# magneano/shyft

Measured on NVIDIA B200. Metric: cell-timesteps/sec (pt_gs_k run_cells), higher is better.
Workload: dtype f64

## Files before the change

### shyft_b200/csrc/sb2_capi.cu

```cuda
#include <cuda_runtime.h>

#include <cstdio>
#include <cstdlib>
#include <cstring>
#include <map>
#include <mutex>
#include <memory>
#include <string>
#include <type_traits>
#include <vector>

#include "../../include/shyft_b200.h"
#include "sb2_host.hpp"
#include "sb2_interp.cuh"
#include "sb2_ptgsk.cuh"
#include "sb2_hbv.cuh"
#include "sb2_ptssk.cuh"
#include "sb2_pthpsk.cuh"
#include "sb2_routing.cuh"
#include <nvtx3/nvToolsExt.h>
#include "sb2_unit.cuh"
#include "sb2_goal.cuh"
#include "sb2_stats.cuh"

// ... 532 lines not shown
        nvtxRangePop();
        m->launches += 3;
    } else {
        const dim3 grid((unsigned)(groups * n_slices), ne);
        zero_tickets();
        if (m->stack == SB2_PT_SS_K) {
            SskRunArgs a{};
            common(a);
            a.params = m->d_ssk_params.p;
            a.inv_dt_hours = make_inv_divisor(a.dt_hours);
            a.step_in_days = a.dt_seconds / 86400.0;
            a.collect = collect & 15;
            ptssk_run_kernel<<<grid, SB2_BLOCK, SB2_MTAB_BYTES, m->stream>>>(a);
        } else if (m->stack == SB2_PT_HPS_K) {
            HpsRunArgs a{};
            common(a);
            a.params = m->d_hps_params.p;
            a.bb0 = 0.98 * 5.670373e-8 * sb_pow4(273.15);
            a.inv_dt_seconds = make_inv_divisor(a.dt_seconds);
            a.ens_params = t.hps_members; a.ens_state_stride = t.state_stride; a.ens_partial_stride = t.partial_stride; a.ens_resp_stride = t.resp_stride;
            a.collect = collect & 15;
            if (t.hps_members) pthpsk_run_kernel<true><<<grid, SB2_BLOCK, SB2_MTAB_BYTES, m->stream>>>(a);
            else pthpsk_run_kernel<false><<<grid, SB2_BLOCK, SB2_MTAB_BYTES, m->stream>>>(a);
        } else {
            HbvRunArgs a{};
            common(a);
            a.params = m->d_hbv_params.p;
            a.inv_dt_hours = make_inv_divisor(a.dt_hours);
            a.step_in_days = a.dt_seconds / 86400.0;
            a.par0 = make_hbv_param(m->stack == SB2_HBV_STACK, m->region_param.data());
            a.ens_params = t.hbv_members; a.ens_state_stride = t.state_stride; a.ens_partial_stride = t.partial_stride; a.ens_resp_stride = t.resp_stride;
            a.collect = collect & 15;
            if (m->stack == SB2_PT_HS_K) {
                if (upar) hbv_run_kernel<false, true><<<grid, SB2_BLOCK, SB2_MTAB_BYTES, m->stream>>>(a);
                else hbv_run_kernel<false, false><<<grid, SB2_BLOCK, SB2_MTAB_BYTES, m->stream>>>(a);
            } else {
                if (upar) hbv_run_kernel<true, true><<<grid, SB2_BLOCK, SB2_MTAB_BYTES, m->stream>>>(a);
                else hbv_run_kernel<true, false><<<grid, SB2_BLOCK, SB2_MTAB_BYTES, m->stream>>>(a);
            }
        }
        ++m->launches;
    }
    CUDA_OK(cudaGetLastError());
    NvtxRange nv_reduce("catchment_reduce");
    const int64_t total = int64_t(chunk) * m->n_catch();
    catchment_reduce_kernel<<<dim3((unsigned)grid_for(total, 256), ne), 256, 0, m->stream>>>(
        t.partial, m->n_slots, m->d_cat_ptr.p, m->d_cat_slots.p, int(m->n_catch()), chunk, t.cq, t.cc, s0, t.partial_stride, t.catch_stride);
    CUDA_OK(cudaGetLastError());
    ++m->launches;
}

void launch_step_range(sb2_model* m, int64_t first, int64_t n_steps, bool collect_end_state) {
    sync_parameters(m);
    sync_filter(m);
    const int64_t n = m->n;
    if (m->partial_steps == 0) {
        constexpr int64_t cap = 4096, scratch_gb = 16;
        int64_t ps = std::max<int64_t>(1, std::min<int64_t>(cap, (int64_t(cap / 4) << 20) / std::max<int64_t>(1, m->n_slots * 16)));
        if (m->stack == SB2_PT_GS_K) ps = std::max<int64_t>(16, std::min<int64_t>(ps, (scratch_gb << 30) / (40 * std::max<int64_t>(1, n))));
        m->partial_steps = int(ps);
        m->d_partial.resize(size_t(ps) * m->n_slots * 2);
    }
    if (m->stack == SB2_PT_GS_K)
        for (auto& b : m->d_scr) b.ensure(size_t(std::min<int64_t>(m->partial_steps, n_steps)) * n);
    m->d_tickets.ensure(size_t(1 + step_groups(m)));
    StepTarget t;
    t.state = m->d_state.p; t.partial = m->d_partial.p; t.cq = m->d_cq.p; t.cc = m->d_cc.p; t.scr = m->d_scr;
    t.tickets = m->d_tickets.p;
    t.series = true;
    const int64_t n_chunks = std::max<int64_t>(1, (n_steps + m->partial_steps - 1) / m->partial_steps);
    int64_t even = (n_steps + n_chunks - 1) / n_chunks;
    even = std::min<int64_t>(m->partial_steps, (even + 127) / 128 * 128);
    for (int64_t done = 0; done < n_steps; done += even) {
        const int chunk = int(std::min<int64_t>(even, n_steps - done));
        launch_step_chunk(m, t, first + done, chunk, collect_end_state && done + chunk >= n_steps);
    }
}

void check_device_errors(sb2_model* m) {
    int flag = 0;
    CUDA_OK(cudaMemcpyAsync(&flag, m->d_error_flag.p, sizeof(int), cudaMemcpyDeviceToHost, m->stream));
    CUDA_OK(cudaStreamSynchronize(m->stream));
    if (flag) {
        CUDA_OK(cudaMemsetAsync(m->d_error_flag.p, 0, sizeof(int), m->stream));
        if (flag & ERR_KIRCHNER_STEP) throw Error("Max number of iterations exceeded (500). A new step size was not found.");
        if (flag & ERR_HBV_NEGATIVE_OUTFLOW) throw Error("hbv_snow: Negative outflow");
        if (flag & ERR_SKAUGEN_SEARCH) throw Error("skaugen: sca_rel_red found no root (boost::math::tools::bisect: no change of sign) or the gamma density overflowed");
        throw Error("device error flag " + std::to_string(flag));
    }
}

void validate_run_args(const sb2_model* m, int start_step, int n_steps) {
    if (!(m->T > 0)) throw Error("region_model::run with invalid time_axis invoked");
    if (start_step < 0 || int64_t(start_step) + 1 > m->T) throw Error("region_model::run start_step must in range[0..n_steps-1>");
    if (n_steps < 0) throw Error("region_model::run n_steps must be range[0..time-axis-steps]");
    if (int64_t(start_step) + n_steps > m->T) throw Error("region_model::run start_step+n_steps must be within time-axis range");
}
void snapshot_initial_state_if_unset(sb2_model* m) {
    if (m->has_initial) return;
    m->d_initial_state.resize(m->d_state.n);
    CUDA_OK(cudaMemcpyAsync(m->d_initial_state.p, m->d_state.p, m->d_state.n * sizeof(double), cudaMemcpyDeviceToDevice, m->stream));
    m->has_initial = true;
}

IdwParam to_idw(const sb2_idw_parameter& q) {
    IdwParam p{};
    p.max_members = int(q.max_members);
    p.max_distance = q.max_distance;
    p.distance_measure_factor = q.distance_measure_factor;
    p.zscale = q.zscale;
    p.default_temp_gradient = q.default_temp_gradient;
    p.scale_factor = q.scale_factor;
    p.gradient_by_equation = q.gradient_by_equation;
    return p;
}
const sb2_idw_parameter& idw_parameter_of(const sb2_interpolation_parameter& ip, int var) {
    switch (var) {
        case SB2_TEMPERATURE: return ip.temperature_idw;
        case SB2_PRECIPITATION: return ip.precipitation;
        case SB2_RADIATION: return ip.radiation;
        case SB2_WIND_SPEED: return ip.wind_speed;
        default: return ip.rel_hum;
    }
}
int idw_kind_of(int var) {
    switch (var) {
        case SB2_TEMPERATURE: return IDW_TEMPERATURE;
        case SB2_PRECIPITATION: return IDW_PRECIPITATION;
        case SB2_RADIATION: return IDW_RADIATION;
        case SB2_WIND_SPEED: return IDW_WIND_SPEED;
        default: return IDW_REL_HUM;
    }
}

void build_idw_plan(sb2_model* m, int var) {
    IdwPlan& pl = m->idw[var];
    const Source& s = m->src[var];
    pl.p = to_idw(idw_parameter_of(m->ip, var));
    if (pl.p.max_members < 1) throw Error("inverse_distance: max_members must be >= 1");
    pl.n_src = s.n_src;
    const size_t k = size_t(std::min<int64_t>(pl.p.max_members, s.n_src));
    pl.idx.resize(k * m->n); pl.w.resize(k * m->n); pl.f.resize(k * m->n); pl.cnt.resize(m->n);
    const double d2 = pl.p.max_distance * pl.p.max_distance;
    const double min_weight = 1.0 / sb_pow(d2, pl.p.distance_measure_factor / 2.0);
    idw_build_neighbours_kernel<<<grid_for(m->n, 128), 128, 0, m->stream>>>(idw_kind_of(var), m->n, m->d_x.p, m->d_y.p, m->d_z.p, m->d_slope.p,
                                                                           int(s.n_src), s.d_xyz.p, pl.p, min_weight, pl.idx.p, pl.w.p, pl.f.p,
                                                                           pl.cnt.p);
    CUDA_OK(cudaGetLastError());
    ++m->launches;
    pl.valid = true;
    pl.dense_valid = false;
}

int idw_tile_steps(int64_t n_src) {
    const int64_t budget = 32 * 1024 / 8;
    return int(std::max<int64_t>(1, std::min<int64_t>(64, budget / std::max<int64_t>(1, n_src))));
}

void run_idw(sb2_model* m, int var, int64_t first, int64_t n_steps, double* out) {
    IdwPlan& pl = m->idw[var];
    if (!pl.valid) build_idw_plan(m, var);
    const Source& s = m->src[var];
    if (!s.has_nonfinite && !(var == SB2_TEMPERATURE && pl.p.gradient_by_equation) && s.n_src <= 96 && !m->force_sparse_idw) {
        if (!pl.dense_valid) {
            pl.dense.resize(size_t(s.n_src) * m->n);
            pl.addc.resize(size_t(m->n));
            idw_build_dense_kernel<<<grid_for(m->n, 128), 128, 0, m->stream>>>(idw_kind_of(var), m->n, int(s.n_src), m->d_z.p, pl.p.default_temp_gradient,
                                                                              pl.idx.p, pl.w.p, pl.f.p, pl.cnt.p, pl.dense.p, pl.addc.p);
            CUDA_OK(cudaGetLastError());
            ++m->launches;
            const int nvp = int(s.n_src);
            const int ks = nvp <= 16 ? 4 : (nvp <= 32 ? 8 : (nvp <= 64 ? 16 : 24)), ntile = nvp <= 32 ? 4 : (nvp <= 64 ? 2 : 1);
            const int64_t n_tiles = grid_for(m->n, 32 * ntile) * 4;
            pl.ulist.resize(size_t(n_tiles) * ks * 4);
            pl.ukc.resize(size_t(n_tiles));
            CUDA_OK(cudaMemsetAsync(pl.ukc.p, 0, size_t(n_tiles), m->stream));
            idw_union_plan_kernel<<<grid_for(n_tiles * 32, 128), 128, 0, m->stream>>>(m->n, nvp, pl.dense.p, 8 * ntile, ks * 4, pl.ulist.p, pl.ukc.p);
            CUDA_OK(cudaGetLastError());
            ++m->launches;
            std::vector<uint8_t> h_kc(size_t(n_tiles), 0);
            CUDA_OK(cudaMemcpyAsync(h_kc.data(), pl.ukc.p, h_kc.size(), cudaMemcpyDeviceToHost, m->stream));
            CUDA_OK(cudaStreamSynchronize(m->stream));
            pl.kc_max = 0;
            for (uint8_t k : h_kc) pl.kc_max = std::max(pl.kc_max, int(k));
            pl.dense_valid = true;
        }
        const int nv = int(s.n_src);
        const double* v = s.d_values.p + first * s.n_src;
        const int use_tma = (nv % 2 == 0 && (reinterpret_cast<uintptr_t>(v) & 15) == 0) ? 1 : 0;
#define SB2_DENSE(KS, NT, KROW, TS)                                                                                                       \
    do {                                                                                                                                  \
        const int smem = dense_smem_bytes(KROW, TS);                                                                                      \
        auto kern = dense_apply_dmma_kernel<KS, NT, 0, true, KROW, TS>;                                                                   \
        CUDA_OK(cudaFuncSetAttribute(kern, cudaFuncAttributeMaxDynamicSharedMemorySize, smem));                                           \
        kern<<<grid_for(m->n, 32 * NT), 128, smem, m->stream>>>(m->n, nullptr, nv, pl.dense.p, pl.addc.p, nullptr, v, s.n_src, nullptr,   \
                                                                int(n_steps), m->d_active.p, out, pl.ulist.p, pl.ukc.p, use_tma,          \
                                                                4 * (nv <= 16 ? 4 : (nv <= 32 ? 8 : (nv <= 64 ? 16 : 24))));              \
    } while (0)
        if (nv <= 16) SB2_DENSE(4, 4, 4, 0);
        else if (nv <= 32) SB2_DENSE(8, 4, 8, 0);
        else if (nv <= 64) {
            if (pl.kc_max <= 4) SB2_DENSE(4, 2, 16, SB2_DENSE_TILE_COMPACT);
            else if (pl.kc_max <= 6) SB2_DENSE(6, 2, 16, SB2_DENSE_TILE_COMPACT);
            else if (pl.kc_max <= 8) SB2_DENSE(8, 2, 16, SB2_DENSE_TILE_COMPACT);
            else if (pl.kc_max <= 10) SB2_DENSE(10, 2, 16, SB2_DENSE_TILE_COMPACT);
            else if (pl.kc_max <= 12) SB2_DENSE(12, 2, 16, SB2_DENSE_TILE_COMPACT);
            else SB2_DENSE(16, 2, 16, 0);
        } else SB2_DENSE(24, 1, 24, 0);
#undef SB2_DENSE
        CUDA_OK(cudaGetLastError());
        ++m->launches;
        return;
    }
    const int tile = idw_tile_steps(s.n_src);
    const int max_k = int(std::max<int64_t>(1, std::min<int64_t>(pl.p.max_members, s.n_src)));
    const size_t smem = size_t(tile) * s.n_src * sizeof(double) + size_t(max_k) * IDW_BLOCK * (2 * sizeof(double) + sizeof(int));
    if (smem > 200 * 1024) throw Error("inverse_distance: too many sources / members for the shared-memory tiles");
    const int g = grid_for(m->n, IDW_BLOCK);
#define SB2_IDW(K)                                                                                                                   \
    {                                                                                                                                \
        if (smem > 48 * 1024) CUDA_OK(cudaFuncSetAttribute(idw_apply_kernel<K>, cudaFuncAttributeMaxDynamicSharedMemorySize, int(smem))); \
        idw_apply_kernel<K><<<g, IDW_BLOCK, smem, m->stream>>>(m->n, m->d_z.p, int(s.n_src), s.d_xyz.p, s.d_values.p, first, int(n_steps),  \
                                                               pl.p, pl.idx.p, pl.w.p, pl.f.p, pl.cnt.p, m->d_active.p, out, tile, max_k);     \
    }
    switch (idw_kind_of(var)) {
        case IDW_TEMPERATURE: SB2_IDW(IDW_TEMPERATURE) break;
        case IDW_PRECIPITATION: SB2_IDW(IDW_PRECIPITATION) break;
        case IDW_RADIATION: SB2_IDW(IDW_RADIATION) break;
        case IDW_WIND_SPEED: SB2_IDW(IDW_WIND_SPEED) break;
        default: SB2_IDW(IDW_REL_HUM) break;
    }
#undef SB2_IDW
    CUDA_OK(cudaGetLastError());
    ++m->launches;
}

BtkOps* btk_ops_for(sb2_model* m, const std::vector<int>& valid, bool check_rank) {
    for (auto& o : m->btk_cache)
        if (o->valid == valid) return o.get();
    if (m->btk_cache.size() >= 8) m->btk_cache.erase(m->btk_cache.begin() + 1);
    const Source& s = m->src[SB2_TEMPERATURE];
    const sb2_btk_parameter& bp = m->ip.temperature;
    host::BtkStationOps h = host::btk_station_ops(s.xyz, valid, bp.sill, bp.nug, bp.range, bp.zscale, bp.gradient_sd, check_rank);
    auto o = std::make_unique<BtkOps>();
    o->valid = valid;
    const int nv = int(valid.size());
    std::vector<double> sub_xyz(size_t(nv) * 3);
    for (int i = 0; i < nv; ++i)
        for (int c = 0; c < 3; ++c) sub_xyz[3 * i + c] = s.xyz[3 * valid[i] + c];
    DevArray<double> d_sub_xyz, d_Kinv, d_FtKinv, d_M22;
    d_sub_xyz.upload(sub_xyz, m->stream);
    d_Kinv.upload(h.K_inv.a, m->stream);
    d_FtKinv.upload(h.FtKinv.a, m->stream);
    d_M22.upload(h.M22.a, m->stream);
    o->E_beta_w.upload(h.E_beta_w.a, m->stream);
    o->sz.upload(h.z, m->stream);
    std::vector<int32_t> vi(valid.begin(), valid.end());
    o->valid_idx.upload(vi, m->stream);
    o->omega.resize(size_t(nv) * m->n);
    o->bm.resize(size_t(2) * m->n);
    m->d_btk_kbuf.ensure(size_t(nv) * m->n);
    btk_build_operators_kernel<<<grid_for(m->n, 128), 128, 0, m->stream>>>(m->n, m->d_x.p, m->d_y.p, m->d_z.p, nv, d_sub_xyz.p, d_Kinv.p,
                                                                          d_FtKinv.p, d_M22.p, bp.sill - bp.nug, bp.range, bp.zscale,
                                                                          o->omega.p, o->bm.p, m->d_btk_kbuf.p);
    CUDA_OK(cudaGetLastError());
    ++m->launches;
    CUDA_OK(cudaStreamSynchronize(m->stream));
    m->btk_cache.push_back(std::move(o));
    return m->btk_cache.back().get();
}

void run_btk(sb2_model* m, int64_t first, int64_t n_steps, double* out) {
    const Source& s = m->src[SB2_TEMPERATURE];
    const int S = int(s.n_src);
    std::vector<int> all(S);
    for (int i = 0; i < S; ++i) all[i] = i;
    BtkOps* full = btk_ops_for(m, all, true);
    int64_t i = 0;
    while (i < n_steps) {
        std::vector<int> valid;
        if (!s.has_nonfinite) valid = all;
        else {
            const double* v = &s.h_values[size_t(first + i) * S];
            for (int k = 0; k < S; ++k) if (std::isfinite(v[k])) valid.push_back(k);
        }
        if (valid.empty()) throw Error("bayesian kriging temperature: No valid sources for time period, giving up.");
        int64_t j = i + 1;
        if (!s.has_nonfinite) j = n_steps;
        else
            for (; j < n_steps; ++j) {
                const double* v = &s.h_values[size_t(first + j) * S];
                bool same = true;
                size_t q = 0;
                for (int k = 0; k < S && same; ++k) {
                    const bool fin = std::isfinite(v[k]);
                    const bool was = q < valid.size() && valid[q] == k;
                    if (fin != was) same = false;
                    if (was) ++q;
                }
                if (!same) break;
            }
        BtkOps* op = int(valid.size()) == S ? full : btk_ops_for(m, valid, false);
        const int nv = int(valid.size());
        const int64_t seg = j - i;
        m->d_btk_beta.ensure(size_t(seg) * 2);
        m->d_btk_resid.ensure(size_t(seg) * nv);
        btk_step_prepare_kernel<<<grid_for(seg, 128), 128, 0, m->stream>>>(int(seg), first + i, S, s.d_values.p, op->valid_idx.p, nv,
                                                                          op->E_beta_w.p, op->sz.p, m->d_btk_beta.p, m->d_btk_resid.p);
        CUDA_OK(cudaGetLastError());
        double* o = out + i * m->n;
        const double* pri = m->d_prior_gradient.p + first + i;
        const int use_tma = (nv % 2 == 0 && (reinterpret_cast<uintptr_t>(m->d_btk_resid.p) & 15) == 0) ? 1 : 0;
#define SB2_BTK(KS, NT, TS)                                                                                                               \
    do {                                                                                                                                  \
        const int smem = dense_smem_bytes(KS, TS);                                                                                        \
        auto kern = dense_apply_dmma_kernel<KS, NT, 1, false, KS, TS>;                                                                    \
        CUDA_OK(cudaFuncSetAttribute(kern, cudaFuncAttributeMaxDynamicSharedMemorySize, smem));                                           \
        kern<<<grid_for(m->n, 32 * NT), 128, smem, m->stream>>>(m->n, m->d_z.p, nv, op->omega.p, op->bm.p, m->d_btk_beta.p,               \
                                                                m->d_btk_resid.p, nv, pri, int(seg), m->d_active.p, o, nullptr, nullptr,  \
                                                                use_tma, 0);                                                              \
    } while (0)
        if (nv <= 16) SB2_BTK(4, 4, 0);
        else if (nv <= 32) SB2_BTK(8, 4, 0);
        else if (nv <= 64) SB2_BTK(16, 2, 0);
        else if (nv <= 96) SB2_BTK(24, 1, 0);
        else {
            const int tile = idw_tile_steps(nv);
            const size_t smem = size_t(tile) * nv * sizeof(double);
            btk_apply_kernel<<<grid_for(m->n, 128), 128, smem, m->stream>>>(m->n, m->d_z.p, nv, op->omega.p, op->bm.p, m->d_btk_beta.p,
                                                                           m->d_btk_resid.p, pri, int(seg), m->d_active.p, o, tile);
        }
#undef SB2_BTK
        CUDA_OK(cudaGetLastError());
        m->launches += 2;
        i = j;
    }
}

void interpolate_variable(sb2_model* m, int var, int64_t first, int64_t n_steps, double* out) {
    const Source& s = m->src[var];
    if (s.n_src == 0) return;
    if (var == SB2_TEMPERATURE) {
        if (s.n_src > 1) {
            if (m->ip.use_idw_for_temperature) run_idw(m, var, first, n_steps, out);
            else run_btk(m, first, n_steps, out);
        } else {
            broadcast_source_kernel<<<grid_for(m->n, 128), 128, 0, m->stream>>>(m->n, s.d_values.p + first, int(n_steps), m->d_active.p, out);
            CUDA_OK(cudaGetLastError());
            ++m->launches;
        }
    } else run_idw(m, var, first, n_steps, out);
}

bool interpolate_range(sb2_model* m, int64_t first, int64_t n_steps, int best_effort) {
    NvtxRange nv("interpolate");
    sync_filter(m);
    bool all_ok = true;
    for (int var = 0; var < SB2_N_FORCING; ++var) {
        try {
            interpolate_variable(m, var, first, n_steps, m->d_forcing[var].p + (first - m->forcing_first) * m->n);
        } catch (const std::exception&) {
            if (!best_effort) throw;
            all_ok = false;
        }
    }
    return all_ok;
}

void set_interpolation_parameter(sb2_model* m, const sb2_interpolation_parameter* ip) {
    if (!ip) throw Error("null interpolation parameter");
    if (m->ip_valid && std::memcmp(&m->ip, ip, sizeof(*ip)) == 0) return;
    m->ip = *ip;
    m->ip_valid = true;
    for (auto& pl : m->idw) pl.valid = false;
    m->btk_cache.clear();
}

void ensure_forcing(sb2_model* m, int64_t first, int64_t rows, bool nan_fill) {
    if (m->forcing_first == first && m->forcing_rows == rows && m->d_forcing[0].p) return;
    for (auto& f : m->d_forcing) f.resize(size_t(rows) * m->n);
    m->forcing_first = first;
    m->forcing_rows = rows;
    if (nan_fill)
        for (auto& f : m->d_forcing) fill_nan(m, f.p, rows * m->n);
}

void copy_out_2d(sb2_model* m, const double* d_src , int64_t rows, double* out, int layout) {
    if (layout == SB2_TIME_MAJOR) {
        CUDA_OK(cudaMemcpyAsync(out, d_src, size_t(rows) * m->n * sizeof(double), cudaMemcpyDeviceToHost, m->stream));
    } else {
        DevArray<double> tmp;
        tmp.resize(size_t(rows) * m->n);
        dim3 b(32, 8), g((unsigned)((m->n + 31) / 32), (unsigned)((rows + 31) / 32));
        transpose_kernel<<<g, b, 0, m->stream>>>(d_src, tmp.p, rows, m->n);
        CUDA_OK(cudaGetLastError());
        ++m->launches;
        CUDA_OK(cudaMemcpyAsync(out, tmp.p, size_t(rows) * m->n * sizeof(double), cudaMemcpyDeviceToHost, m->stream));
        CUDA_OK(cudaStreamSynchronize(m->stream));
        return;
    }
    CUDA_OK(cudaStreamSynchronize(m->stream));
}

void time_begin(sb2_model* m, int which) { CUDA_OK(cudaEventRecord(m->ev[which], m->stream)); }
float time_end(sb2_model* m, int a, int b) {
    CUDA_OK(cudaEventRecord(m->ev[b], m->stream));
    CUDA_OK(cudaEventSynchronize(m->ev[b]));
    float ms = 0.f;
    CUDA_OK(cudaEventElapsedTime(&ms, m->ev[a], m->ev[b]));
    return ms;
}
void ensure_routing_plan(sb2_model* m) {
    if (m->route) return;
    if (m->rivers.empty()) throw Error("routing: the river network is empty");
    const int off = kStacks[m->stack].routing_velocity;
    std::vector<double> cell_routing(size_t(m->n) * 5);
    for (int64_t i = 0; i < m->n; ++i) {
        auto f = m->catch_param.find(m->geo[i].catchment_id);
        const std::vector<double>& p = f != m->catch_param.end() ? f->second : m->region_param;
        double* cr = &cell_routing[5 * i];
        cr[0] = double(m->geo[i].routing_id); cr[1] = m->geo[i].routing_distance;
        cr[2] = p[off]; cr[3] = p[off + 1]; cr[4] = p[off + 2];
    }
    m->route = build_routing_plan(m->rivers, cell_routing, m->n, m->dt, m->stream);
}


void build_goal_targets(sb2_model* m, std::vector<GoalTarget>& gt, const double* cq, const double* cc, int64_t ens_stride) {
    gt.clear();
    int first_kind = -1;
    for (auto& tp : m->targets)
        if (first_kind < 0 && (tp->property == SB2_TARGET_DISCHARGE || tp->property == SB2_TARGET_CELL_CHARGE)) first_kind = tp->property;
    for (auto& tp : m->targets) {
        sb2_model::Target& t = *tp;
        GoalTarget g{};
        g.obs = t.d_obs.p;
        g.first_step = (t.t0 - m->t0) / m->dt;
        g.steps_per_period = int32_t(t.dt / m->dt);
        g.n = int32_t(t.obs.size());
        g.calc_mode = (t.calc_mode == SB2_GOAL_ABS_DIFF && t.property == SB2_TARGET_CELL_CHARGE) ? GOAL_ABS_DIFF_SCALED : t.calc_mode;
        g.s_r = t.s_r; g.s_a = t.s_a; g.s_b = t.s_b;
        g.dt_seconds = double(m->dt) / 1e6;
        g.rows = m->T;
        g.scale = nullptr;
        if (t.property == SB2_TARGET_DISCHARGE || t.property == SB2_TARGET_CELL_CHARGE) {
            g.series = first_kind == SB2_TARGET_DISCHARGE ? cq : cc;
            g.ens_stride = ens_stride;
            g.n_col = int32_t(m->n_catch());
            g.cix = t.d_cix.p;
            g.n_cix = int32_t(t.cids.size());
        } else {
            g.series = t.d_series.p;
            g.ens_stride = 0;
            g.n_col = 1;
            g.cix = t.d_cix.p;
            g.n_cix = 1;
        }
        if (!t.aligned) {
            if (ens_stride != 0) throw Error("target_specification: batched evaluation needs target axes aligned with the model axis");
            const int64_t T = m->T, n = int64_t(t.obs.size());
            if (!m->d_axis_t.p || int64_t(m->d_axis_t.n) != T) {
                std::vector<int64_t> tt(static_cast<size_t>(T), 0);
                for (int64_t i = 0; i < T; ++i) tt[size_t(i)] = m->t0 + i * m->dt;
                m->d_axis_t.upload(tt, m->stream);
            }
            DevArray<double> d_prop, d_a, d_b;
            d_prop.resize(size_t(T));
            t.d_projected.resize(size_t(n));
            auto project = [&](int mode, double* out) {
                goal_property_kernel<<<grid_for(T, 256), 256, 0, m->stream>>>(g.series, T, g.n_col, g.cix, g.n_cix, mode, d_prop.p);
                if (t.points.empty())
                    average_accessor_kernel<<<grid_for(n, 256), 256, 0, m->stream>>>(m->d_axis_t.p, d_prop.p, T, 1, m->t0 + T * m->dt, 0, t.t0, t.dt, n, out);
                else
// ... 1400 lines not shown
```

### shyft_b200/csrc/sb2_interp.cuh

```cuda
#pragma once
#include <stdint.h>

#include "sb2_math.cuh"

namespace sb2 {

enum { IDW_TEMPERATURE = 0, IDW_PRECIPITATION = 1, IDW_RADIATION = 2, IDW_WIND_SPEED = 3, IDW_REL_HUM = 4 };

struct IdwParam {
    int max_members;
    double max_distance, distance_measure_factor, zscale, default_temp_gradient, scale_factor;
    int gradient_by_equation;
};

__device__ __forceinline__ double distance_measure(double ax, double ay, double az, double bx, double by, double bz, double p, double zscale) {
    const double dx = __dsub_rn(ax, bx), dy = __dsub_rn(ay, by), dz = __dsub_rn(az, bz);
    const double d2 = __dadd_rn(__dadd_rn(__dmul_rn(dx, dx), __dmul_rn(dy, dy)), __dmul_rn(__dmul_rn(__dmul_rn(dz, dz), zscale), zscale));
    const double e = p / 2.0;
    return sb_pow(d2, e);
}

__global__ void idw_build_neighbours_kernel(int kind, int64_t n_cells, const double* __restrict__ cx, const double* __restrict__ cy,
                                            const double* __restrict__ cz, const double* __restrict__ cslope, int n_src,
                                            const double* __restrict__ sxyz, IdwParam p, double min_weight, int32_t* __restrict__ nb_idx,
// ... 82 lines not shown
    double* sf = sw + (size_t)max_k * IDW_BLOCK;
    int* sk = (int*)(sf + (size_t)max_k * IDW_BLOCK);
    const int tid = threadIdx.x;
    const int64_t c = (int64_t)blockIdx.x * blockDim.x + tid;
    const bool ok = c < n_cells && (active == nullptr || active[c] != 0);
    const int cnt = ok ? nb_n[c] : 0;
    const double z = ok ? cz[c] : 0.0;
    for (int j = 0; j < cnt; ++j) {
        sk[j * IDW_BLOCK + tid] = nb_idx[(int64_t)j * n_cells + c];
        sw[j * IDW_BLOCK + tid] = nb_w[(int64_t)j * n_cells + c];
        sf[j * IDW_BLOCK + tid] = nb_f[(int64_t)j * n_cells + c];
    }
    for (int t0 = 0; t0 < n_steps; t0 += tile_steps) {
        const int nt = min(tile_steps, n_steps - t0);
        __syncthreads();
        for (int e = tid; e < nt * n_src; e += blockDim.x) sv[e] = src[(first_step + t0) * n_src + e];
        __syncthreads();
        if (!ok) continue;
        for (int i = 0; i < nt; ++i) {
            const double* v = sv + i * n_src;
            double scale = 1.0;
            if (KIND == IDW_TEMPERATURE) {
                scale = p.default_temp_gradient;
                int nv = 0, mn = -1, mx = -1, first[4] = {-1, -1, -1, -1};
                double zmn = 0, zmx = 0;
                for (int j = 0; j < cnt; ++j) {
                    const int k = sk[j * IDW_BLOCK + tid];
                    if (!isfinite(v[k])) continue;
                    const double h = sf[j * IDW_BLOCK + tid];
                    if (nv < 4) first[nv] = k;
                    if (nv == 0) { mn = mx = k; zmn = zmx = h; }
                    else if (h < zmn) { mn = k; zmn = h; }
                    else if (h > zmx) { mx = k; zmx = h; }
                    ++nv;
                }
                bool solved = false;
                if (p.gradient_by_equation && nv > 3) {
                    double A[3][3], b[3], x[3];
                    for (int r = 0; r < 3; ++r) {
                        A[r][0] = sxyz[3 * first[r + 1]] - sxyz[3 * first[0]];
                        A[r][1] = sxyz[3 * first[r + 1] + 1] - sxyz[3 * first[0] + 1];
                        A[r][2] = sxyz[3 * first[r + 1] + 2] - sxyz[3 * first[0] + 2];
                        b[r] = v[first[r + 1]] - v[first[0]];
                    }
                    if (solve3(A, b, x)) { scale = x[2]; solved = true; }
                }
                if (!solved && nv > 1) {
                    const double dz = zmx - zmn;
                    scale = dz > 50.0 ? (v[mx] - v[mn]) / dz : p.default_temp_gradient;
                }
            }
            double sum_w = 0, sum_wv = 0;
            for (int j = 0; j < cnt; ++j) {
                const double s = v[sk[j * IDW_BLOCK + tid]];
                if (isfinite(s)) {
                    const double w = sw[j * IDW_BLOCK + tid];
                    double tv;
                    if (KIND == IDW_TEMPERATURE) tv = s + scale * (z - sf[j * IDW_BLOCK + tid]);
                    else if (KIND == IDW_PRECIPITATION || KIND == IDW_RADIATION) tv = s * sf[j * IDW_BLOCK + tid];
                    else tv = s;
                    sum_wv += w * tv;
                    sum_w += w;
                }
            }
            out[(int64_t)(t0 + i) * n_cells + c] = sum_wv / sum_w;
        }
    }
}

__global__ void btk_build_operators_kernel(int64_t n_cells, const double* __restrict__ cx, const double* __restrict__ cy,
                                           const double* __restrict__ cz, int n_src, const double* __restrict__ sxyz,
                                           const double* __restrict__ K_inv, const double* __restrict__ FtKinv,
                                           const double* __restrict__ M22, double sill_m_nug, double range, double zscale,
                                           double* __restrict__ omega , double* __restrict__ bm ,
                                           double* __restrict__ kbuf ) {
    const int64_t c = (int64_t)blockIdx.x * blockDim.x + threadIdx.x;
    if (c >= n_cells) return;
    const double x = cx[c], y = cy[c], z = cz[c];
    for (int s = 0; s < n_src; ++s) {
        const double dx = sxyz[3 * s] - x, dy = sxyz[3 * s + 1] - y, dz = sxyz[3 * s + 2] - z;
        const double d = sqrt(dx * dx + dy * dy + dz * dz * zscale * zscale);
        kbuf[(int64_t)s * n_cells + c] = sill_m_nug * sb_exp(-d / range);
    }
    double g0 = 0.0, g1 = 0.0;
    for (int j = 0; j < n_src; ++j) {
        const double kj = kbuf[(int64_t)j * n_cells + c];
        g0 += FtKinv[j] * kj;
        g1 += FtKinv[n_src + j] * kj;
    }
    const double d0 = 1.0 - g0, d1 = z - g1;
    bm[c] = d0 * M22[0] + d1 * M22[2];
    bm[n_cells + c] = d0 * M22[1] + d1 * M22[3];
    for (int s = 0; s < n_src; ++s) {
        double acc = 0.0;
        for (int j = 0; j < n_src; ++j) acc += kbuf[(int64_t)j * n_cells + c] * K_inv[j * n_src + s];
        omega[(int64_t)s * n_cells + c] = acc;
    }
}

__global__ void btk_step_prepare_kernel(int n_steps, int64_t first_step, int n_src, const double* __restrict__ src,
                                        const int32_t* __restrict__ valid_idx, int n_valid, const double* __restrict__ E_beta_w ,
                                        const double* __restrict__ sz_valid, double* __restrict__ beta ,
                                        double* __restrict__ resid ) {
    const int i = blockIdx.x * blockDim.x + threadIdx.x;
    if (i >= n_steps) return;
    const double* v = src + (first_step + i) * n_src;
    double b0 = 0.0, b1 = 0.0;
    for (int s = 0; s < n_valid; ++s) {
        const double t = v[valid_idx[s]];
        b0 += E_beta_w[s] * t;
        b1 += E_beta_w[n_valid + s] * t;
    }
    beta[2 * i] = b0;
    beta[2 * i + 1] = b1;
    for (int s = 0; s < n_valid; ++s) resid[(int64_t)i * n_valid + s] = v[valid_idx[s]] - (1.0 * b0 + sz_valid[s] * b1);
}

__global__ void __launch_bounds__(128) btk_apply_kernel(int64_t n_cells, const double* __restrict__ cz, int n_valid,
                                                        const double* __restrict__ omega , const double* __restrict__ bm,
                                                        const double* __restrict__ beta, const double* __restrict__ resid,
                                                        const double* __restrict__ prior_gradient , int n_steps,
                                                        const uint8_t* __restrict__ active, double* __restrict__ out ,
                                                        int tile_steps) {
    extern __shared__ double sr[];
    const int64_t c = (int64_t)blockIdx.x * blockDim.x + threadIdx.x;
    const bool ok = c < n_cells && (active == nullptr || active[c] != 0);
    const double z = ok ? cz[c] : 0.0, bm0 = ok ? bm[c] : 0.0, bm1 = ok ? bm[n_cells + c] : 0.0;
    for (int t0 = 0; t0 < n_steps; t0 += tile_steps) {
        const int nt = min(tile_steps, n_steps - t0);
        __syncthreads();
        for (int e = threadIdx.x; e < nt * n_valid; e += blockDim.x) sr[e] = resid[(int64_t)t0 * n_valid + e];
        __syncthreads();
        if (!ok) continue;
        for (int i = 0; i < nt; ++i) {
            const double b0 = beta[2 * (t0 + i)], b1 = beta[2 * (t0 + i) + 1];
            double acc = 0.0;
            for (int s = 0; s < n_valid; ++s) acc += omega[(int64_t)s * n_cells + c] * sr[i * n_valid + s];
            const double t_hat = (1.0 * b0 + z * b1) + acc;
            out[(int64_t)(t0 + i) * n_cells + c] = t_hat - (bm0 * (b0 - 0.0) + bm1 * (b1 - prior_gradient[t0 + i]));
        }
    }
}

__device__ __forceinline__ void dmma_m8n8k4(double& d0, double& d1, double a, double b) {
    asm volatile("mma.sync.aligned.m8n8k4.row.col.f64.f64.f64.f64 {%0,%1}, {%2}, {%3}, {%0,%1};" : "+d"(d0), "+d"(d1) : "d"(a), "d"(b));
}
__device__ __forceinline__ uint32_t smem_u32(const void* p) { return (uint32_t)__cvta_generic_to_shared(p); }
__device__ __forceinline__ void mbar_init(unsigned long long* bar, int count) {
    asm volatile("mbarrier.init.shared::cta.b64 [%0], %1;" ::"r"(smem_u32(bar)), "r"(count));
}
__device__ __forceinline__ void mbar_arrive_expect_tx(unsigned long long* bar, uint32_t bytes) {
    asm volatile("mbarrier.arrive.expect_tx.shared::cta.b64 _, [%0], %1;" ::"r"(smem_u32(bar)), "r"(bytes) : "memory");
}
__device__ __forceinline__ void bulk_copy_g2s(void* dst, const void* src, uint32_t bytes, unsigned long long* bar) {
    asm volatile("cp.async.bulk.shared::cluster.global.mbarrier::complete_tx::bytes [%0], [%1], %2, [%3];" ::"r"(smem_u32(dst)), "l"(src), "r"(bytes),
                 "r"(smem_u32(bar))
                 : "memory");
}
__device__ __forceinline__ void mbar_wait(unsigned long long* bar, uint32_t parity) {
    uint32_t done = 0;
    for (int spins = 0; !done; ++spins) {
        asm volatile("{\n.reg .pred p;\nmbarrier.try_wait.parity.shared::cta.b64 p, [%1], %2;\nselp.u32 %0, 1, 0, p;\n}" : "=r"(done) : "r"(smem_u32(bar)), "r"(parity) : "memory");
        if (spins > (1 << 24)) __trap();
    }
}

__host__ __device__ constexpr int dense_tile_steps(int krow, int tile_steps) { return tile_steps > 0 ? tile_steps : (krow > 16 ? 32 : 64); }
__host__ __device__ constexpr int dense_smem_bytes(int krow, int tile_steps) { return 2 * dense_tile_steps(krow, tile_steps) * (krow * 4 + 4) * 8; }
template <int KSTEPS, int NT, int MODE, bool COMPACT, int KROW = KSTEPS, int TILE_STEPS = 0>
__global__ void __launch_bounds__(128) dense_apply_dmma_kernel(int64_t n_cells, const double* __restrict__ cz, int n_valid,
                                                               const double* __restrict__ omega , const double* __restrict__ bm,
                                                               const double* __restrict__ beta ,
                                                               const double* __restrict__ resid , int64_t row_stride,
                                                               const double* __restrict__ prior_gradient , int n_steps,
                                                               const uint8_t* __restrict__ active, double* __restrict__ out ,
                                                               const int32_t* __restrict__ ulist, const uint8_t* __restrict__ ukc, int use_tma,
                                                               int ul_stride ) {
    constexpr int KP = KROW * 4 + 4;
    constexpr int TILE = dense_tile_steps(KROW, TILE_STEPS);
    extern __shared__ __align__(16) double sr_dyn[];
    __shared__ double sbeta[2][TILE * 2];
    __shared__ double spri[2][TILE];
    __shared__ __align__(8) unsigned long long bar[2];
    const int lane = threadIdx.x & 31, warp = threadIdx.x >> 5;
    const int g = lane >> 2, q = lane & 3;
    const int64_t tile = (int64_t)blockIdx.x * 4 + warp;
    const int64_t cbase = tile * (8 * NT);
    int ul[KSTEPS];
#pragma unroll
    for (int ks = 0; ks < KSTEPS; ++ks) ul[ks] = COMPACT ? ulist[tile * ul_stride + ks * 4 + q] : ks * 4 + q;
    const int kc = COMPACT ? min(int(ukc[tile]), KSTEPS) : KSTEPS;
    double breg[NT][KSTEPS];
#pragma unroll
    for (int nt = 0; nt < NT; ++nt) {
        const int64_t cell = cbase + nt * 8 + g;
#pragma unroll
        for (int ks = 0; ks < KSTEPS; ++ks) {
            const int st = ul[ks];
            breg[nt][ks] = (cell < n_cells && st < n_valid) ? omega[(int64_t)st * n_cells + cell] : 0.0;
        }
    }
    double ez[NT][2], e0[NT][2], e1[NT][2];
    bool eok[NT][2];
#pragma unroll
    for (int nt = 0; nt < NT; ++nt)
#pragma unroll
        for (int h = 0; h < 2; ++h) {
            const int64_t cell = cbase + nt * 8 + q * 2 + h;
            const bool ok = cell < n_cells && (active == nullptr || active[cell] != 0);
            eok[nt][h] = ok;
            if (MODE == 1) {
                ez[nt][h] = ok ? cz[cell] : 0.0;
                e0[nt][h] = ok ? bm[cell] : 0.0;
                e1[nt][h] = ok ? bm[n_cells + cell] : 0.0;
            } else {
                ez[nt][h] = (ok && bm != nullptr) ? bm[cell] : 0.0;
                e0[nt][h] = e1[nt][h] = 0.0;
            }
        }
    for (int e = threadIdx.x; e < 2 * TILE * KP; e += blockDim.x) sr_dyn[e] = 0.0;
    if (threadIdx.x == 0 && use_tma) { mbar_init(&bar[0], 1); mbar_init(&bar[1], 1); }
    asm volatile("fence.proxy.async.shared::cta;" ::: "memory");
    __syncthreads();
    const int n_tiles = (n_steps + TILE - 1) / TILE;
    const bool vec_ok = (n_cells % 2 == 0) && ((reinterpret_cast<uintptr_t>(out) & 15) == 0);
    auto stage = [&](int it) {
        const int buf = it & 1, t0 = it * TILE;
        const int nt_steps = min(TILE, n_steps - t0);
        double* dst = sr_dyn + buf * TILE * KP;
        if (use_tma) {
            if (warp == 0) {
                if (lane == 0) mbar_arrive_expect_tx(&bar[buf], (uint32_t)(nt_steps * n_valid * 8));
                __syncwarp();
                for (int r = lane; r < nt_steps; r += 32)
                    bulk_copy_g2s(dst + r * KP, resid + (int64_t)(t0 + r) * row_stride, (uint32_t)(n_valid * 8), &bar[buf]);
            }
        } else {
            for (int e = threadIdx.x; e < TILE * n_valid; e += blockDim.x) {
                const int r = e / n_valid, k = e - r * n_valid;
                dst[r * KP + k] = r < nt_steps ? resid[(int64_t)(t0 + r) * row_stride + k] : 0.0;
            }
        }
        if (MODE == 1)
            for (int e = threadIdx.x; e < TILE; e += blockDim.x) {
                const bool in = e < nt_steps;
                sbeta[buf][2 * e] = in ? beta[2 * (t0 + e)] : 0.0;
                sbeta[buf][2 * e + 1] = in ? beta[2 * (t0 + e) + 1] : 0.0;
                spri[buf][e] = in ? prior_gradient[t0 + e] : 0.0;
            }
    };
    stage(0);
    for (int it = 0; it < n_tiles; ++it) {
        const int buf = it & 1, t0 = it * TILE;
        const int nt_steps = min(TILE, n_steps - t0);
        if (it + 1 < n_tiles) stage(it + 1);
        if (use_tma) mbar_wait(&bar[buf], (uint32_t)((it >> 1) & 1));
        __syncthreads();
        const double* sr = sr_dyn + buf * TILE * KP;
        for (int m0 = 0; m0 < nt_steps; m0 += 8) {
            double acc[NT][2];
#pragma unroll
            for (int nt = 0; nt < NT; ++nt) acc[nt][0] = acc[nt][1] = 0.0;
#pragma unroll
            for (int ks = 0; ks < KSTEPS; ++ks) {
                if (!COMPACT || ks < kc) {
                    const double a = sr[(m0 + g) * KP + ul[ks]];
#pragma unroll
                    for (int nt = 0; nt < NT; ++nt) dmma_m8n8k4(acc[nt][0], acc[nt][1], a, breg[nt][ks]);
                }
            }
            const int tl = m0 + g;
            if (tl < nt_steps) {
                double b0 = 0.0, b1 = 0.0, pri = 0.0;
                if (MODE == 1) { b0 = sbeta[buf][2 * tl]; b1 = sbeta[buf][2 * tl + 1]; pri = spri[buf][tl]; }
#pragma unroll
                for (int nt = 0; nt < NT; ++nt) {
                    double v[2];
#pragma unroll
                    for (int h = 0; h < 2; ++h) {
                        if (MODE == 1) {
                            const double t_hat = (1.0 * b0 + ez[nt][h] * b1) + acc[nt][h];
                            v[h] = t_hat - (e0[nt][h] * (b0 - 0.0) + e1[nt][h] * (b1 - pri));
                        } else
                            v[h] = acc[nt][h] + ez[nt][h];
                    }
                    double* dst = out + (int64_t)(t0 + tl) * n_cells + cbase + nt * 8 + q * 2;
                    if (eok[nt][0] && eok[nt][1] && vec_ok) *reinterpret_cast<double2*>(dst) = make_double2(v[0], v[1]);
                    else {
                        if (eok[nt][0]) dst[0] = v[0];
                        if (eok[nt][1]) dst[1] = v[1];
                    }
                }
            }
        }
        __syncthreads();
    }
}

__global__ void idw_build_dense_kernel(int kind, int64_t n_cells, int n_src, const double* __restrict__ cz, double default_gradient,
                                       const int32_t* __restrict__ nb_idx, const double* __restrict__ nb_w, const double* __restrict__ nb_f,
                                       const int32_t* __restrict__ nb_n, double* __restrict__ W , double* __restrict__ addc) {
    const int64_t c = (int64_t)blockIdx.x * blockDim.x + threadIdx.x;
    if (c >= n_cells) return;
    for (int s = 0; s < n_src; ++s) W[(int64_t)s * n_cells + c] = 0.0;
    const int cnt = nb_n[c];
    addc[c] = 0.0;
    if (cnt == 0) { W[c] = nan_(); return; }
    double sum_w = 0.0;
    for (int j = 0; j < cnt; ++j) sum_w += nb_w[(int64_t)j * n_cells + c];
    for (int j = 0; j < cnt; ++j) {
        const int k = nb_idx[(int64_t)j * n_cells + c];
        const double w = nb_w[(int64_t)j * n_cells + c];
        const double f = (kind == IDW_PRECIPITATION || kind == IDW_RADIATION) ? nb_f[(int64_t)j * n_cells + c] : 1.0;
        W[(int64_t)k * n_cells + c] += w * f / sum_w;
    }
    if (kind == IDW_TEMPERATURE) {
        int mn = -1, mx = -1;
        double zmn = 0, zmx = 0, zbar = 0.0;
        for (int j = 0; j < cnt; ++j) {
            const int k = nb_idx[(int64_t)j * n_cells + c];
            const double h = nb_f[(int64_t)j * n_cells + c];
            zbar += nb_w[(int64_t)j * n_cells + c] * h;
            if (j == 0) { mn = mx = k; zmn = zmx = h; }
            else if (h < zmn) { mn = k; zmn = h; }
            else if (h > zmx) { mx = k; zmx = h; }
        }
        zbar /= sum_w;
        const double dz = zmx - zmn, lever = cz[c] - zbar;
        if (cnt > 1 && dz > 50.0) {
            W[(int64_t)mx * n_cells + c] += lever / dz;
            W[(int64_t)mn * n_cells + c] -= lever / dz;
        } else
            addc[c] = default_gradient * lever;
    }
}

__global__ void idw_union_plan_kernel(int64_t n_cells, int n_src, const double* __restrict__ W , int cells_per_tile,
                                      int k_slots, int32_t* __restrict__ ulist , uint8_t* __restrict__ ukc) {
    const int64_t tile = ((int64_t)blockIdx.x * blockDim.x + threadIdx.x) >> 5;
    const int lane = threadIdx.x & 31;
    const int64_t n_tiles = (n_cells + cells_per_tile - 1) / cells_per_tile;
    if (tile >= n_tiles) return;
    const int64_t cell = tile * cells_per_tile + lane;
    const bool mine = lane < cells_per_tile && cell < n_cells;
    int count = 0;
    for (int s = 0; s < n_src; ++s) {
        const bool nz = mine && W[(int64_t)s * n_cells + cell] != 0.0;
        if (__any_sync(0xffffffffu, nz)) {
            if (lane == 0) ulist[tile * k_slots + count] = s;
            ++count;
        }
    }
    for (int k = count + lane; k < k_slots; k += 32) ulist[tile * k_slots + k] = k_slots;
    if (lane == 0) ukc[tile] = (uint8_t)((count + 3) / 4);
}

__global__ void fill_kernel(double* __restrict__ p, int64_t n, double v) {
    for (int64_t i = (int64_t)blockIdx.x * blockDim.x + threadIdx.x; i < n; i += (int64_t)gridDim.x * blockDim.x) p[i] = v;
}
__global__ void average_accessor_same_axis_kernel(double* __restrict__ p, int64_t n, double dt_seconds, int* __restrict__ nonfinite) {
    bool bad = false;
    for (int64_t i = (int64_t)blockIdx.x * blockDim.x + threadIdx.x; i < n; i += (int64_t)gridDim.x * blockDim.x) {
        const double v = p[i];
        const bool fin = isfinite(v);
        bad |= !fin;
        p[i] = fin ? (dt_seconds * v) / dt_seconds : nan("");
    }
    if (bad) atomicOr(nonfinite, 1);
}
__device__ __forceinline__ double us_to_seconds(int64_t us) { return double(us) / 1000000.0; }
__device__ __forceinline__ double average_accessor_value(const int64_t* __restrict__ t , const double* __restrict__ values ,
                                                         int64_t v_stride, int64_t n_points, int64_t t_end, int linear, int64_t p_start, int64_t p_end) {
    const double nan_v = nan_();
    double result = nan_v;
    if (n_points > 0 && p_start < t_end) {
        int64_t i = 0;
        if (!(p_start < t[0])) {
            int64_t lo = 0, hi = n_points;
            while (hi - lo > 1) {
                const int64_t mid = (lo + hi) >> 1;
                if (t[mid] <= p_start) lo = mid; else hi = mid;
            }
            i = lo;
        }
        const bool extrapolate_flat = !linear;
        int64_t l_t = 0, tsum = 0;
        double l_v = 0.0, area = 0.0;
        bool l_finite = false;
        while (true) {
            if (!l_finite) {
                l_t = t[i]; l_v = values[i * v_stride]; ++i;
                l_finite = isfinite(l_v);
                if (i == n_points) {
                    if (l_finite && l_t < p_end && extrapolate_flat) {
                        const int64_t dt = p_end - (p_start > l_t ? p_start : l_t);
                        tsum += dt;
                        area += us_to_seconds(dt) * l_v;
                    }
                    break;
                }
                if (l_t >= p_end) break;
            } else {
                const int64_t r_t = t[i];
                const double r_v = values[i * v_stride];
                ++i;
                const bool r_finite = isfinite(r_v);
                const int64_t px_start = l_t > p_start ? l_t : p_start, px_end = r_t < p_end ? r_t : p_end;
                int64_t dt = px_end - px_start;
                if (linear && r_finite) {
                    const double a = (r_v - l_v) / us_to_seconds(r_t - l_t);
                    const double b = r_v - a * us_to_seconds(r_t);
                    area += us_to_seconds(dt) * (0.5 * a * us_to_seconds(px_start + px_end) + b);
                    tsum += dt;
                } else if (extrapolate_flat) {
                    area += l_v * us_to_seconds(dt);
                    tsum += dt;
                }
                if (i == n_points) {
                    if (r_finite && r_t < p_end && extrapolate_flat) {
                        dt = p_end - r_t;
                        tsum += dt;
                        area += us_to_seconds(dt) * r_v;
                    }
                    break;
                }
                if (r_t >= p_end) break;
                l_finite = r_finite;
                l_t = r_t;
                l_v = r_v;
            }
        }
        result = tsum > 0 ? area / us_to_seconds(tsum) : nan_v;
    }
    return result;
}

__global__ void average_accessor_kernel(const int64_t* __restrict__ t , const double* __restrict__ values ,
                                        int64_t n_points, int64_t n_src, int64_t t_end, int linear, int64_t ta_t0, int64_t ta_dt, int64_t ta_n,
                                        double* __restrict__ out ) {
    const int64_t idx = (int64_t)blockIdx.x * blockDim.x + threadIdx.x;
    if (idx >= ta_n * n_src) return;
    const int64_t step = idx / n_src, s = idx - step * n_src;
    const int64_t p_start = ta_t0 + step * ta_dt;
    out[idx] = average_accessor_value(t, values + s, n_src, n_points, t_end, linear, p_start, p_start + ta_dt);
}
__global__ void average_accessor_periods_kernel(const int64_t* __restrict__ t, const double* __restrict__ values, int64_t n_points, int64_t t_end,
                                                int linear, const int64_t* __restrict__ pts , int64_t n, double* __restrict__ out) {
    const int64_t i = (int64_t)blockIdx.x * blockDim.x + threadIdx.x;
// ... 64 lines not shown
```

Measured before the change: 9.860 billion.

## Make dense DMMA apply kernel persistent with 3-stage mbarrier producer/consumer pipeline

The dense IDW/BTK apply kernel becomes persistent. The grid is sized from occupancy times SM count, and each block walks a contiguous range of (cell-tile, time-tile) work units. Block-wide __syncthreads double buffering is replaced by a 3-stage ring of full/empty mbarriers, where the last warp to release a stage refills it. This is meant to overlap loads with compute and avoid whole-block barriers, at the cost of reloading omega and cell coefficients whenever the cell tile changes and added barrier complexity. The default tile is also fixed at 32 steps, and launch bounds are tightened for one BTK variant.

```diff
diff --git a/shyft_b200/csrc/sb2_capi.cu b/shyft_b200/csrc/sb2_capi.cu
--- a/shyft_b200/csrc/sb2_capi.cu
+++ b/shyft_b200/csrc/sb2_capi.cu
@@ -708,6 +708,15 @@
     pl.dense_valid = false;
 }
 
+template <typename K>
+int dense_grid(const sb2_model* m, K kern, int smem, int cells_per_block, int64_t n_steps, int tile_steps) {
+    int per_sm = 0, sms = 0;
+    CUDA_OK(cudaOccupancyMaxActiveBlocksPerMultiprocessor(&per_sm, kern, 32 * DENSE_WARPS, smem));
+    CUDA_OK(cudaDeviceGetAttribute(&sms, cudaDevAttrMultiProcessorCount, m->device));
+    const int64_t units = ((m->n + cells_per_block - 1) / cells_per_block) * ((n_steps + tile_steps - 1) / tile_steps);
+    return int(std::max<int64_t>(1, std::min<int64_t>(int64_t(std::max(per_sm, 1)) * sms, units)));
+}
+
 int idw_tile_steps(int64_t n_src) {
     const int64_t budget = 32 * 1024 / 8;
     return int(std::max<int64_t>(1, std::min<int64_t>(64, budget / std::max<int64_t>(1, n_src))));
@@ -749,9 +758,10 @@
         const int smem = dense_smem_bytes(KROW, TS);                                                                                      \
         auto kern = dense_apply_dmma_kernel<KS, NT, 0, true, KROW, TS>;                                                                   \
         CUDA_OK(cudaFuncSetAttribute(kern, cudaFuncAttributeMaxDynamicSharedMemorySize, smem));                                           \
-        kern<<<grid_for(m->n, 32 * NT), 128, smem, m->stream>>>(m->n, nullptr, nv, pl.dense.p, pl.addc.p, nullptr, v, s.n_src, nullptr,   \
-                                                                int(n_steps), m->d_active.p, out, pl.ulist.p, pl.ukc.p, use_tma,          \
-                                                                4 * (nv <= 16 ? 4 : (nv <= 32 ? 8 : (nv <= 64 ? 16 : 24))));              \
+        const int grid = dense_grid(m, kern, smem, 32 * NT, n_steps, dense_tile_steps(KROW, TS));                                       \
+        kern<<<grid, 32 * DENSE_WARPS, smem, m->stream>>>(m->n, nullptr, nv, pl.dense.p, pl.addc.p, nullptr, v, s.n_src, nullptr,         \
+                                                          int(n_steps), m->d_active.p, out, pl.ulist.p, pl.ukc.p, use_tma,                \
+                                                          4 * (nv <= 16 ? 4 : (nv <= 32 ? 8 : (nv <= 64 ? 16 : 24))));                    \
     } while (0)
         if (nv <= 16) SB2_DENSE(4, 4, 4, 0);
         else if (nv <= 32) SB2_DENSE(8, 4, 8, 0);
@@ -872,9 +882,10 @@
         const int smem = dense_smem_bytes(KS, TS);                                                                                        \
         auto kern = dense_apply_dmma_kernel<KS, NT, 1, false, KS, TS>;                                                                    \
         CUDA_OK(cudaFuncSetAttribute(kern, cudaFuncAttributeMaxDynamicSharedMemorySize, smem));                                           \
-        kern<<<grid_for(m->n, 32 * NT), 128, smem, m->stream>>>(m->n, m->d_z.p, nv, op->omega.p, op->bm.p, m->d_btk_beta.p,               \
-                                                                m->d_btk_resid.p, nv, pri, int(seg), m->d_active.p, o, nullptr, nullptr,  \
-                                                                use_tma, 0);                                                              \
+        const int grid = dense_grid(m, kern, smem, 32 * NT, seg, dense_tile_steps(KS, TS));                                            \
+        kern<<<grid, 32 * DENSE_WARPS, smem, m->stream>>>(m->n, m->d_z.p, nv, op->omega.p, op->bm.p, m->d_btk_beta.p,                     \
+                                                          m->d_btk_resid.p, nv, pri, int(seg), m->d_active.p, o, nullptr, nullptr,        \
+                                                          use_tma, 0);                                                                    \
     } while (0)
         if (nv <= 16) SB2_BTK(4, 4, 0);
         else if (nv <= 32) SB2_BTK(8, 4, 0);
diff --git a/shyft_b200/csrc/sb2_interp.cuh b/shyft_b200/csrc/sb2_interp.cuh
--- a/shyft_b200/csrc/sb2_interp.cuh
+++ b/shyft_b200/csrc/sb2_interp.cuh
@@ -258,6 +258,19 @@
 __device__ __forceinline__ void mbar_arrive_expect_tx(unsigned long long* bar, uint32_t bytes) {
     asm volatile("mbarrier.arrive.expect_tx.shared::cta.b64 _, [%0], %1;" ::"r"(smem_u32(bar)), "r"(bytes) : "memory");
 }
+__device__ __forceinline__ void mbar_arrive(unsigned long long* bar) {
+    asm volatile("mbarrier.arrive.shared::cta.b64 _, [%0];" ::"r"(smem_u32(bar)) : "memory");
+}
+__device__ __forceinline__ bool mbar_arrive_last(unsigned long long* bar, uint32_t parity) {
+    uint32_t pending;
+    asm volatile("{\n.reg .b64 st;\nmbarrier.arrive.shared::cta.b64 st, [%1];\nmbarrier.pending_count.b64 %0, st;\n}"
+                 : "=r"(pending) : "r"(smem_u32(bar)) : "memory");
+    if (pending != 1) return false;
+    uint32_t done = 0;
+    while (!done)
+        asm volatile("{\n.reg .pred p;\nmbarrier.try_wait.parity.shared::cta.b64 p, [%1], %2;\nselp.u32 %0, 1, 0, p;\n}" : "=r"(done) : "r"(smem_u32(bar)), "r"(parity) : "memory");
+    return true;
+}
 __device__ __forceinline__ void bulk_copy_g2s(void* dst, const void* src, uint32_t bytes, unsigned long long* bar) {
     asm volatile("cp.async.bulk.shared::cluster.global.mbarrier::complete_tx::bytes [%0], [%1], %2, [%3];" ::"r"(smem_u32(dst)), "l"(src), "r"(bytes),
                  "r"(smem_u32(bar))
@@ -271,10 +284,18 @@
     }
 }
 
-__host__ __device__ constexpr int dense_tile_steps(int krow, int tile_steps) { return tile_steps > 0 ? tile_steps : (krow > 16 ? 32 : 64); }
-__host__ __device__ constexpr int dense_smem_bytes(int krow, int tile_steps) { return 2 * dense_tile_steps(krow, tile_steps) * (krow * 4 + 4) * 8; }
+#ifndef SB2_DENSE_TILE_X
+#define SB2_DENSE_TILE_X 0
+#endif
+#ifndef SB2_DENSE_STAGES_X
+#define SB2_DENSE_STAGES_X 3
+#endif
+__host__ __device__ constexpr int dense_tile_steps(int krow, int tile_steps) { return SB2_DENSE_TILE_X > 0 ? SB2_DENSE_TILE_X : (tile_steps > 0 ? tile_steps : 32); }
+constexpr int DENSE_STAGES = SB2_DENSE_STAGES_X;
+constexpr int DENSE_WARPS = 4;
+__host__ __device__ constexpr int dense_smem_bytes(int krow, int tile_steps) { return DENSE_STAGES * dense_tile_steps(krow, tile_steps) * (krow * 4 + 4) * 8; }
 template <int KSTEPS, int NT, int MODE, bool COMPACT, int KROW = KSTEPS, int TILE_STEPS = 0>
-__global__ void __launch_bounds__(128) dense_apply_dmma_kernel(int64_t n_cells, const double* __restrict__ cz, int n_valid,
+__global__ void __launch_bounds__(32 * DENSE_WARPS, MODE == 1 && KSTEPS == 16 ? 4 : 0) dense_apply_dmma_kernel(int64_t n_cells, const double* __restrict__ cz, int n_valid,
                                                                const double* __restrict__ omega , const double* __restrict__ bm,
                                                                const double* __restrict__ beta ,
                                                                const double* __restrict__ resid , int64_t row_stride,
@@ -284,85 +305,97 @@
                                                                int ul_stride ) {
     constexpr int KP = KROW * 4 + 4;
     constexpr int TILE = dense_tile_steps(KROW, TILE_STEPS);
+    constexpr int NS = DENSE_STAGES;
     extern __shared__ __align__(16) double sr_dyn[];
-    __shared__ double sbeta[2][TILE * 2];
-    __shared__ double spri[2][TILE];
-    __shared__ __align__(8) unsigned long long bar[2];
+    __shared__ double sbeta[NS][MODE == 1 ? TILE * 2 : 1];
+    __shared__ double spri[NS][MODE == 1 ? TILE : 1];
+    __shared__ __align__(8) unsigned long long full[NS];
+    __shared__ __align__(8) unsigned long long empty[NS];
     const int lane = threadIdx.x & 31, warp = threadIdx.x >> 5;
     const int g = lane >> 2, q = lane & 3;
-    const int64_t tile = (int64_t)blockIdx.x * 4 + warp;
-    const int64_t cbase = tile * (8 * NT);
-    int ul[KSTEPS];
-#pragma unroll
-    for (int ks = 0; ks < KSTEPS; ++ks) ul[ks] = COMPACT ? ulist[tile * ul_stride + ks * 4 + q] : ks * 4 + q;
-    const int kc = COMPACT ? min(int(ukc[tile]), KSTEPS) : KSTEPS;
-    double breg[NT][KSTEPS];
-#pragma unroll
-    for (int nt = 0; nt < NT; ++nt) {
-        const int64_t cell = cbase + nt * 8 + g;
-#pragma unroll
-        for (int ks = 0; ks < KSTEPS; ++ks) {
-            const int st = ul[ks];
-            breg[nt][ks] = (cell < n_cells && st < n_valid) ? omega[(int64_t)st * n_cells + cell] : 0.0;
-        }
-    }
-    double ez[NT][2], e0[NT][2], e1[NT][2];
-    bool eok[NT][2];
-#pragma unroll
-    for (int nt = 0; nt < NT; ++nt)
-#pragma unroll
-        for (int h = 0; h < 2; ++h) {
-            const int64_t cell = cbase + nt * 8 + q * 2 + h;
-            const bool ok = cell < n_cells && (active == nullptr || active[cell] != 0);
-            eok[nt][h] = ok;
-            if (MODE == 1) {
-                ez[nt][h] = ok ? cz[cell] : 0.0;
-                e0[nt][h] = ok ? bm[cell] : 0.0;
-                e1[nt][h] = ok ? bm[n_cells + cell] : 0.0;
-            } else {
-                ez[nt][h] = (ok && bm != nullptr) ? bm[cell] : 0.0;
-                e0[nt][h] = e1[nt][h] = 0.0;
-            }
-        }
-    for (int e = threadIdx.x; e < 2 * TILE * KP; e += blockDim.x) sr_dyn[e] = 0.0;
-    if (threadIdx.x == 0 && use_tma) { mbar_init(&bar[0], 1); mbar_init(&bar[1], 1); }
+    const int n_st = (n_steps + TILE - 1) / TILE;
+    const int64_t n_ct = (n_cells + 32 * NT - 1) / (32 * NT);
+    const int64_t u_all = n_ct * n_st;
+    const int64_t u0 = u_all * blockIdx.x / gridDim.x;
+    const int n_units = int(u_all * (blockIdx.x + 1) / gridDim.x - u0);
+    for (int e = threadIdx.x; e < NS * TILE * KP; e += blockDim.x) sr_dyn[e] = 0.0;
+    if (threadIdx.x < NS) { mbar_init(&full[threadIdx.x], 1); mbar_init(&empty[threadIdx.x], DENSE_WARPS); }
     asm volatile("fence.proxy.async.shared::cta;" ::: "memory");
     __syncthreads();
-    const int n_tiles = (n_steps + TILE - 1) / TILE;
-    const bool vec_ok = (n_cells % 2 == 0) && ((reinterpret_cast<uintptr_t>(out) & 15) == 0);
-    auto stage = [&](int it) {
-        const int buf = it & 1, t0 = it * TILE;
+    auto fill = [&](int k, int stf) {
+        const int s = k % NS;
+        const int t0 = stf * TILE;
         const int nt_steps = min(TILE, n_steps - t0);
-        double* dst = sr_dyn + buf * TILE * KP;
+        double* dst = sr_dyn + s * TILE * KP;
+        if (MODE == 1)
+            for (int e = lane; e < TILE; e += 32) {
+                const bool in = e < nt_steps;
+                sbeta[s][2 * e] = in ? beta[2 * (t0 + e)] : 0.0;
+                sbeta[s][2 * e + 1] = in ? beta[2 * (t0 + e) + 1] : 0.0;
+                spri[s][e] = in ? prior_gradient[t0 + e] : 0.0;
+            }
         if (use_tma) {
-            if (warp == 0) {
-                if (lane == 0) mbar_arrive_expect_tx(&bar[buf], (uint32_t)(nt_steps * n_valid * 8));
-                __syncwarp();
-                for (int r = lane; r < nt_steps; r += 32)
-                    bulk_copy_g2s(dst + r * KP, resid + (int64_t)(t0 + r) * row_stride, (uint32_t)(n_valid * 8), &bar[buf]);
-            }
+            __syncwarp();
+            if (lane == 0) mbar_arrive_expect_tx(&full[s], (uint32_t)(nt_steps * n_valid * 8));
+            __syncwarp();
+            for (int r = lane; r < nt_steps; r += 32)
+                bulk_copy_g2s(dst + r * KP, resid + (int64_t)(t0 + r) * row_stride, (uint32_t)(n_valid * 8), &full[s]);
         } else {
-            for (int e = threadIdx.x; e < TILE * n_valid; e += blockDim.x) {
+            for (int e = lane; e < TILE * n_valid; e += 32) {
                 const int r = e / n_valid, k = e - r * n_valid;
                 dst[r * KP + k] = r < nt_steps ? resid[(int64_t)(t0 + r) * row_stride + k] : 0.0;
             }
-        }
-        if (MODE == 1)
-            for (int e = threadIdx.x; e < TILE; e += blockDim.x) {
-                const bool in = e < nt_steps;
-                sbeta[buf][2 * e] = in ? beta[2 * (t0 + e)] : 0.0;
-                sbeta[buf][2 * e + 1] = in ? beta[2 * (t0 + e) + 1] : 0.0;
-                spri[buf][e] = in ? prior_gradient[t0 + e] : 0.0;
-            }
+            __syncwarp();
+            if (lane == 0) mbar_arrive(&full[s]);
+        }
     };
-    stage(0);
-    for (int it = 0; it < n_tiles; ++it) {
-        const int buf = it & 1, t0 = it * TILE;
+    if (warp == 0)
+        for (int k = 0; k < min(NS, n_units); ++k) fill(k, int((u0 + k) % n_st));
+    const bool vec_ok = (n_cells % 2 == 0) && ((reinterpret_cast<uintptr_t>(out) & 15) == 0);
+    int64_t ct = u0 / n_st;
+    int st = int(u0 - ct * n_st), k = 0;
+    for (; k < n_units; st = 0, ++ct) {
+        {
+            const int64_t tile = ct * DENSE_WARPS + warp;
+            const int64_t cbase = tile * (8 * NT);
+            int ul[KSTEPS];
+#pragma unroll
+            for (int ks = 0; ks < KSTEPS; ++ks) ul[ks] = COMPACT ? ulist[tile * ul_stride + ks * 4 + q] : ks * 4 + q;
+            const int kc = COMPACT ? min(int(ukc[tile]), KSTEPS) : KSTEPS;
+            double breg[NT][KSTEPS];
+#pragma unroll
+            for (int nt = 0; nt < NT; ++nt) {
+                const int64_t cell = cbase + nt * 8 + g;
+#pragma unroll
+                for (int ks = 0; ks < KSTEPS; ++ks) {
+                    const int sn = ul[ks];
+                    breg[nt][ks] = (cell < n_cells && sn < n_valid) ? omega[(int64_t)sn * n_cells + cell] : 0.0;
+                }
+            }
+            double ez[NT][2], e0[NT][2], e1[NT][2];
+            bool eok[NT][2];
+#pragma unroll
+            for (int nt = 0; nt < NT; ++nt)
+#pragma unroll
+                for (int h = 0; h < 2; ++h) {
+                    const int64_t cell = cbase + nt * 8 + q * 2 + h;
+                    const bool ok = cell < n_cells && (active == nullptr || active[cell] != 0);
+                    eok[nt][h] = ok;
+                    if (MODE == 1) {
+                        ez[nt][h] = ok ? cz[cell] : 0.0;
+                        e0[nt][h] = ok ? bm[cell] : 0.0;
+                        e1[nt][h] = ok ? bm[n_cells + cell] : 0.0;
+                    } else {
+                        ez[nt][h] = (ok && bm != nullptr) ? bm[cell] : 0.0;
+                        e0[nt][h] = e1[nt][h] = 0.0;
+                    }
+                }
+            for (const int k_end = min(n_units, k + (n_st - st)); k < k_end; ++k, ++st) {
+        const int buf = k % NS, t0 = st * TILE;
         const int nt_steps = min(TILE, n_steps - t0);
-        if (it + 1 < n_tiles) stage(it + 1);
-        if (use_tma) mbar_wait(&bar[buf], (uint32_t)((it >> 1) & 1));
-        __syncthreads();
+        mbar_wait(&full[buf], (uint32_t)((k / NS) & 1));
         const double* sr = sr_dyn + buf * TILE * KP;
+#pragma unroll 1
         for (int m0 = 0; m0 < nt_steps; m0 += 8) {
             double acc[NT][2];
 #pragma unroll
@@ -399,7 +432,12 @@
                 }
             }
         }
-        __syncthreads();
+        __syncwarp();
+        uint32_t last = 0;
+        if (lane == 0) last = mbar_arrive_last(&empty[buf], (uint32_t)((k / NS) & 1));
+        if (__shfl_sync(0xffffffffu, last, 0) && k + NS < n_units) fill(k + NS, (st + NS) % n_st);
+            }
+        }
     }
 }
 
```

Result: no change. 9.809 billion (median of 6 runs) (-0.5%).
